# rhasspy/piper

Measured on AMD Instinct MI355X. Metric: audio samples/sec, higher is better.
Workload: dtype f32; 1 GPU; BASELINE configs[1]: medium VITS voice (22050 Hz), 1 utterance(s) x 128 phoneme ids per step per GPU, scales 0.667/1.0/0.8; step = inferSeconds span: host ids in (pe_upload) + pe_run, engine draws both noise sites + int16 PCM to host (pe_fetch); parallelism=utterance-parallel x1, one process per GPU, RCCL weight broadcast

## Files before the change

__graft_entry__.py:

```python
import os
import subprocess
import sys

ROOT = os.path.dirname(os.path.abspath(__file__))
if ROOT not in sys.path:
    sys.path.insert(0, ROOT)


def build() -> None:
    subprocess.check_call(["make", "-C", ROOT, "-j", str(min(8, os.cpu_count() or 1)), "all"])
    try:
        subprocess.check_call(["make", "-C", ROOT, "-j", str(min(8, os.cpu_count() or 1)), "emu"])
    except Exception as e:
        print("emulator build skipped:", e)
    import piper_amd
    from piper_amd import _lib
    lib = _lib.get_lib()
    for s in _lib.SYMBOLS:
        getattr(lib, s)


def smoke() -> None:
    import numpy as np
    from oracle import vits_oracle as O
    from piper_amd import weights as W
    from piper_amd.engine import Engine

    cfg = W.preset("tiny")
    w = W.synthetic_weights(cfg, 1234)
    eng = Engine(blob=W.pack_blob(cfg, w), device=0)
    T = 24
    ids = W.synthetic_phoneme_ids(T, 0, id_max=cfg.n_vocab - 1)
    rng = np.random.default_rng(7)
    nw = rng.standard_normal((2, T)).astype(np.float32)
    nz = rng.standard_normal((cfg.inter, 32 * T + 64)).astype(np.float32)
    scales = (0.667, 1.0, 0.8)
    r = eng.synthesize(ids, scales, noise_w=nw, noise_z=nz)
    o = O.synthesize(w, cfg, ids, scales, nw, nz)
    assert np.array_equal(eng.durations(), o["durations"]), "integer durations differ from the oracle"
    d = (r.pcm[0].astype(np.float64) - o["pcm"].astype(np.float64)) / 32767.0
    rms = float(np.sqrt(np.mean(d * d)))
    assert rms <= 1e-3, f"int16 PCM RMS error {rms} > 1e-3"
    print(f"smoke OK: {r.pcm[0].size} samples, pcm rms err {rms:.2e}")


if __name__ == "__main__":
    build()
    if len(sys.argv) > 1 and sys.argv[1] == "smoke":
        smoke()
```

piper_amd/csrc/kernels/col4.h:

```cpp
#pragma once
#include "dds.h"

namespace pe {

__device__ __forceinline__ int c4_tile(int bx, int nx, int P) { return pe_xcd_tile(bx, nx, P); }

constexpr int FFN_MAXS = 16;
constexpr int C4_H = 192, C4_NT = C4_H / 64;
template <int K>
struct Col4W {
  static constexpr int NQ = K / 16;
  static constexpr int KS = K + 4;
  f32x4 w[C4_NT][K / 16];
};
template <int K>
__device__ __forceinline__ void col_gemm4_fetch(Col4W<K>& W, const float* wp4, int nt, int wv, int lane) {
  constexpr int NQ = Col4W<K>::NQ, tile_floats = (K / 4) * 256;
#pragma unroll
  for (int m = 0; m < C4_NT; ++m) {
    const bool live = PE_UNIFORM(m < nt);
    const pe_rowsrc ws = pe_make_row_u(wp4 + (long)(live ? m : 0) * tile_floats, live ? tile_floats : 0);
#pragma unroll
    for (int q = 0; q < NQ; ++q) W.w[m][q] = pe_row_load4(ws, ((NQ * wv + q) * 64 + lane) * 4);
  }
  PE_SCHED_FENCE();
}
template <int K>
__device__ __forceinline__ void col_gemm4_acc(const Col4W<K>& W, const float* YT, f32x4 (&acc)[C4_NT], int wv, int lane) {
  constexpr int NQ = Col4W<K>::NQ, KS = Col4W<K>::KS;
  const float* yp = YT + (lane & 3) * KS + 4 * NQ * wv;
#pragma unroll
  for (int q = 0; q < NQ; ++q) {
    f32x4 yv;
#pragma unroll
    for (int j = 0; j < 4; ++j) yv[j] = yp[4 * q + j];
#pragma unroll
    for (int j = 0; j < 4; ++j)
#pragma unroll
      for (int m = 0; m < C4_NT; ++m) acc[m] = pe_mfma_4x4x1(W.w[m][q][j], yv[j], acc[m]);
  }
}
__device__ __forceinline__ void col_gemm4_zero(f32x4 (&acc)[C4_NT]) {
#pragma unroll
  for (int m = 0; m < C4_NT; ++m)
#pragma unroll
    for (int r = 0; r < 4; ++r) acc[m][r] = 0.f;
}
__device__ __forceinline__ void col_gemm4_put(const f32x4 (&acc)[C4_NT], float* P, int wv, int lane) {
#pragma unroll
  for (int m = 0; m < C4_NT; ++m)
#pragma unroll
    for (int r = 0; r < 4; ++r) P[((wv * C4_NT + m) * 64 + 4 * (lane >> 2) + r) * 4 + (lane & 3)] = acc[m][r];
}
template <int K>
__device__ __forceinline__ void col_gemm4_run(const Col4W<K>& W, const float* YT, float* P, int wv, int lane) {
  f32x4 acc[C4_NT];
  col_gemm4_zero(acc);
  col_gemm4_acc<K>(W, YT, acc, wv, lane);
  col_gemm4_put(acc, P, wv, lane);
}
template <int K, int K2>
__device__ __forceinline__ void col_gemm4_run2(const Col4W<K>& W, const float* YT, const Col4W<K2>& W2, const float* YT2, float* P,
                                               int wv, int lane) {
  f32x4 acc[C4_NT];
  col_gemm4_zero(acc);
  col_gemm4_acc<K>(W, YT, acc, wv, lane);
  col_gemm4_acc<K2>(W2, YT2, acc, wv, lane);
  col_gemm4_put(acc, P, wv, lane);
}
__device__ __forceinline__ float col_gemm4_get(const float* P, int c, int col) {
  const int o = c * 4 + col;
  return ((P[o] + P[C4_H * 4 + o]) + P[2 * C4_H * 4 + o]) + P[3 * C4_H * 4 + o];
}
__device__ __forceinline__ float pe_col_sum4(float v, float* red, int& flip, int wv, int lane, int col) {
  v += __shfl_xor(v, 4);
  v += __shfl_xor(v, 8);
  v += __shfl_xor(v, 16);
  v += __shfl_xor(v, 32);
  float* r = red + flip * 16;
  flip ^= 1;
  if (lane < 4) r[wv * 4 + col] = v;
  __syncthreads();
  return ((r[col] + r[4 + col]) + r[8 + col]) + r[12 + col];
}


template <bool FRONT>
__global__ __launch_bounds__(256) void colchain4_kernel(const int* lens, const float* in1, long in1_bs, int nx, int xcd, int mode,
                                                        int in1_cs, int K1r, int rows1, int first, int out_cs, ColP p) {
  PE_KTRACE(3);
  constexpr int NC = 4, NVT = 3, K1 = C4_H, K2 = C4_H / 2, KS1 = Col4W<K1>::KS, KS2 = Col4W<K2>::KS;
  PE_DYN_SMEM(float, sm);
  if constexpr (!FRONT) PE_STAMP(3, 0);
  p.lens = lens; p.xcd = xcd; p.mode = mode; p.in1 = in1; p.in1_bs = in1_bs; p.in1_cs = in1_cs; p.K1 = K1r; p.rows1 = rows1;
  p.first = first; p.out_cs = out_cs;
  const int b = blockIdx.y;
  int L = PE_UNIFORM(lens[b]);
  if constexpr (FRONT) PE_ENTRY_BATCH(L, p.res, p.res_bs, p.res_cs, p.gamma, p.beta, p.out, p.out_bs, p.x1, p.x1_bs, p.x1_cs, p.b1, p.w1,
                                      p.in0, p.in0_bs, p.in0_cs, p.w0, p.b0, p.w2, p.b2, p.rows2, p.out2, p.o2_bs, p.o2_cs);
  else PE_ENTRY_BATCH(L, p.res, p.res_bs, p.res_cs, p.gamma, p.beta, p.out, p.out_bs, p.x1, p.x1_bs, p.x1_cs, p.b1, p.w1,
                      p.in0, p.in0_bs, p.in0_cs, p.w2, p.b2, p.kT, p.kt_bs, p.vQ);
  const int t0 = c4_tile(blockIdx.x, nx, p.xcd) * NC;
  if (t0 >= L) return;
  if constexpr (!FRONT) PE_STAMP(3, 1);
  float* YT = sm;
  float* P = YT + NC * KS1;
  float* red = P + 4 * C4_H * NC;
  const int tid = threadIdx.x, col = tid & 3, rl = tid >> 2, wv = PE_UNIFORM(tid >> 6), lane = tid & 63;
  const int t = t0 + col;
  const bool ok = t < L;
  const int part = p.mode >= 2 ? (int)blockIdx.z : 0, row0 = part * C4_H;
  const int rows_here = p.rows1 - row0 < C4_H ? p.rows1 - row0 : C4_H;
  const bool nomain = p.mode == 1 && !p.w1;
  Col4W<K1> gw0;
  Col4W<K1> gw;
  auto fetch_gw = [&]() { col_gemm4_fetch<K1>(gw, p.w1 + (long)part * C4_NT * (K1 / 4) * 256, (rows_here + 63) / 64, wv, lane); };
  const bool skip_part = p.mode == 2 && (p.rows1 <= C4_H || part == 1);
  const bool pre_part = !FRONT && p.mode == 2 && p.w2 && !skip_part;
  float* YTP = P + 4 * C4_H * NC + 32 + 64 * 4;
  Col4W<K2> gw2;
  const bool second = p.mode == 1 && p.w2;
  auto chain_tail = [&](auto m_of, const float* ovv) {
    float* xb = p.x1 + (long)b * p.x1_bs;
    float* YT2 = YT;
    const pe_rowsrc b2d = pe_make_row(second ? p.b2 : p.w1, (second && p.b2) ? p.rows2 : 0);
    float b2v[NVT];
#pragma unroll
    for (int k = 0; k < NVT; ++k) b2v[k] = pe_row_load(b2d, rl + 64 * k);
#pragma unroll
    for (int k = 0; k < NVT; ++k) {
      const int c = rl + 64 * k;
      if (c < K2) {
        const float xn = (ok && c < p.rows1) ? ovv[k] - m_of(k, c) : 0.f;
        if (ok && c < p.rows1) xb[(long)c * p.x1_cs + t] = xn;
        YT2[col * KS2 + c] = xn;
      }
    }
    if (!second) return;
    __syncthreads();
    col_gemm4_run<K2>(gw2, YT2, P, wv, lane);
    __syncthreads();
    if (!ok) return;
    float* o2 = p.out2 + (long)b * p.o2_bs;
#pragma unroll
    for (int k = 0; k < NVT; ++k) {
      const int c = rl + 64 * k;
      if (c < p.rows2) o2[(long)c * p.o2_cs + t] = col_gemm4_get(P, c, col) + b2v[k];
    }
  };
  if (nomain) {
    const pe_rowsrc s0 = pe_make_row(p.in1 + (long)b * p.in1_bs, (FRONT && p.first) ? 0 : K2 * p.in1_cs);
    const pe_rowsrc x1d = pe_make_row(p.x1 + (long)b * p.x1_bs, K2 * p.x1_cs);
    float m[NVT], ovn[NVT];
    m[2] = ovn[2] = 0.f;
    if constexpr (FRONT) {
      const pe_rowsrc a0 = pe_make_row(p.in0 + (long)b * p.in0_bs, K1 * p.in0_cs);
      const pe_rowsrc b0d = pe_make_row(p.b0 ? p.b0 : p.w0, p.b0 ? K2 : 0);
      float av[NVT], b0v[2];
#pragma unroll
      for (int k = 0; k < NVT; ++k) av[k] = pe_row_load(a0, ok ? (rl + 64 * k) * p.in0_cs + t : -1);
#pragma unroll
      for (int k = 0; k < 2; ++k) {
        const int c = rl + 64 * k;
        m[k] = pe_row_load(s0, (ok && c < K2) ? c * p.in1_cs + t : -1);
        b0v[k] = pe_row_load(b0d, c);
        ovn[k] = pe_row_load(x1d, (ok && c < K2) ? c * p.x1_cs + t : -1);
      }
      PE_SCHED_FENCE();
      col_gemm4_fetch<K1>(gw0, p.w0, (K2 + 63) / 64, wv, lane);
#pragma unroll
      for (int k = 0; k < NVT; ++k) YT[col * KS1 + rl + 64 * k] = av[k];
      __syncthreads();
      if (second) col_gemm4_fetch<K2>(gw2, p.w2, (p.rows2 + 63) / 64, wv, lane);
      col_gemm4_run<K1>(gw0, YT, P, wv, lane);
      __syncthreads();
#pragma unroll
      for (int k = 0; k < 2; ++k) m[k] = ok ? (col_gemm4_get(P, rl + 64 * k, col) + b0v[k]) + m[k] : 0.f;
    } else {
#pragma unroll
      for (int k = 0; k < 2; ++k) {
        const int c = rl + 64 * k;
        m[k] = pe_row_load(s0, (ok && c < K2) ? c * p.in1_cs + t : -1);
        ovn[k] = pe_row_load(x1d, (ok && c < K2) ? c * p.x1_cs + t : -1);
      }
      PE_SCHED_FENCE();
      if (second) col_gemm4_fetch<K2>(gw2, p.w2, (p.rows2 + 63) / 64, wv, lane);
    }
    chain_tail([&](int k, int) { return m[k]; }, ovn);
    return;
  }
  float sk[NVT];
  if constexpr (FRONT) {
    const pe_rowsrc a0 = pe_make_row(p.in0 + (long)b * p.in0_bs, K1 * p.in0_cs);
    const pe_rowsrc s0 = pe_make_row(p.in1 + (long)b * p.in1_bs, p.first ? 0 : K1 * p.in1_cs);
    const pe_rowsrc b0d = pe_make_row(p.b0 ? p.b0 : p.w0, p.b0 ? K1 : 0);
    float av[NVT], b0v[NVT];
#pragma unroll
    for (int k = 0; k < NVT; ++k) {
      const int c = rl + 64 * k;
      av[k] = pe_row_load(a0, ok ? c * p.in0_cs + t : -1);
      sk[k] = pe_row_load(s0, ok ? c * p.in1_cs + t : -1);
      b0v[k] = pe_row_load(b0d, c);
    }
    PE_SCHED_FENCE();
    col_gemm4_fetch<K1>(gw0, p.w0, C4_NT, wv, lane);
#pragma unroll
    for (int k = 0; k < NVT; ++k) YT[col * KS1 + rl + 64 * k] = av[k];
    __syncthreads();
    fetch_gw();
    col_gemm4_run<K1>(gw0, YT, P, wv, lane);
    __syncthreads();
#pragma unroll
    for (int k = 0; k < NVT; ++k) sk[k] = ok ? (col_gemm4_get(P, rl + 64 * k, col) + b0v[k]) + sk[k] : 0.f;
  }

  float ov[NVT], gg[NVT], bb[NVT], b1v[NVT];
  {
    const pe_rowsrc ind = pe_make_row(p.in1 + (long)b * p.in1_bs, p.K1 * p.in1_cs);
    const float* obp = p.mode == 0 ? p.res + (long)b * p.res_bs : (skip_part ? p.out + (long)b * p.out_bs : p.x1 + (long)b * p.x1_bs);
    const int ocs = p.mode == 0 ? p.res_cs : (skip_part ? p.out_cs : p.x1_cs);
    const pe_rowsrc od = p.mode == 3 ? pe_make_row(p.res ? p.res + (long)b * p.res_bs + row0 : p.w1, p.res ? rows_here : 0)
                         : pre_part  ? pe_make_row(p.b2 ? p.b2 : p.w1, p.b2 ? rows_here : 0)
                                     : pe_make_row(obp, (skip_part && p.first) ? 0 : rows_here * ocs);
    const pe_rowsrc x0d = pe_make_row(p.in0 + (long)b * p.in0_bs, pre_part ? K2 * p.in0_cs : 0);
    float x0v[2];
    const pe_rowsrc gd = pe_make_row(p.mode == 0 ? p.gamma : p.w1, p.mode == 0 ? p.rows1 : 0);
    const pe_rowsrc bd = pe_make_row(p.mode == 0 ? p.beta : p.w1, p.mode == 0 ? p.rows1 : 0);
    const pe_rowsrc b1d = pe_make_row(p.b1 ? p.b1 + row0 : p.w1, p.b1 ? rows_here : 0);
    float xin[NVT];
#pragma unroll
    for (int k = 0; k < NVT; ++k) {
      const int c = rl + 64 * k;
      xin[k] = FRONT ? sk[k] : pe_row_load(ind, ok ? c * p.in1_cs + t : -1);
      ov[k] = pe_row_load(od, (ok && c < rows_here) ? ((p.mode == 3 || pre_part) ? c : c * ocs + t) : -1);
      if (!FRONT && k < 2) x0v[k] = pe_row_load(x0d, (ok && c < K2) ? c * p.in0_cs + t : -1);
      gg[k] = pe_row_load(gd, c < rows_here ? c : -1);
      bb[k] = pe_row_load(bd, c < rows_here ? c : -1);
      b1v[k] = pe_row_load(b1d, c < rows_here ? c : -1);
    }
    PE_SCHED_FENCE();
    if constexpr (!FRONT) fetch_gw();
    if (pre_part) col_gemm4_fetch<K2>(gw2, p.w2, C4_NT, wv, lane);
    if constexpr (!FRONT) PE_STAMP(3, 2);
#pragma unroll
    for (int k = 0; k < NVT; ++k) YT[col * KS1 + rl + 64 * k] = xin[k];
    if constexpr (!FRONT)
      if (pre_part) {
        YTP[col * KS2 + rl] = x0v[0];
        if (rl < K2 - 64) YTP[col * KS2 + rl + 64] = x0v[1];
      }
  }
  __syncthreads();
  if (pre_part) col_gemm4_run2<K1, K2>(gw, YT, gw2, YTP, P, wv, lane);
  else col_gemm4_run<K1>(gw, YT, P, wv, lane);
  if (second) col_gemm4_fetch<K2>(gw2, p.w2, (p.rows2 + 63) / 64, wv, lane);
  __syncthreads();

  if (p.mode >= 2) {
    if (!ok) return;
    float* tp = (skip_part || p.mode == 3) ? p.out + (long)b * p.out_bs + (p.mode == 3 ? (long)row0 * p.out_cs : 0) : p.x1 + (long)b * p.x1_bs;
    const int tcs = (skip_part || p.mode == 3) ? p.out_cs : p.x1_cs;
#pragma unroll
    for (int k = 0; k < NVT; ++k) {
      const int c = rl + 64 * k;
      if (c < rows_here) {
        const float val = (col_gemm4_get(P, c, col) + b1v[k]) + ov[k];
        tp[(long)c * tcs + t] = val;
        if (p.mode == 3 && p.kT && part == 1) p.kT[(long)b * p.kt_bs + ((long)(c >> 2) * p.out_cs + t) * 4 + (c & 3)] = val;
        if (p.mode == 3 && p.vQ && part == 2) p.vQ[(long)b * p.kt_bs + ((long)(t >> 2) * C4_H + c) * 4 + (t & 3)] = val;
      }
    }
    return;
  }
  if (p.mode == 0) {
    int red_flip = 0;
    auto col_sum = [&](float x) -> float { return pe_col_sum4(x, red, red_flip, wv, lane, col); };
    const int H = p.rows1;
    float v[NVT];
    float s = 0.f;
#pragma unroll
    for (int k = 0; k < NVT; ++k) {
      const int c = rl + 64 * k;
      v[k] = (ok && c < H) ? (col_gemm4_get(P, c, col) + b1v[k]) + ov[k] : 0.f;
      s += v[k];
    }
    const float mean = col_sum(s) / (float)H;
    float q = 0.f;
#pragma unroll
    for (int k = 0; k < NVT; ++k)
      if (rl + 64 * k < H) { const float d = v[k] - mean; q = fmaf(d, d, q); }
    const float rstd = 1.f / sqrtf(col_sum(q) / (float)H + 1e-5f);
    if (!ok) return;
    float* ob = p.out + (long)b * p.out_bs;
#pragma unroll
    for (int k = 0; k < NVT; ++k) {
      const int c = rl + 64 * k;
      if (c < H) ob[(long)c * p.out_cs + t] = (v[k] - mean) * rstd * gg[k] + bb[k];
    }
    return;
  }

  chain_tail([&](int k, int c) { return col_gemm4_get(P, c, col) + b1v[k]; }, ov);
}

__global__ __launch_bounds__(256) void lngemm4_kernel(const int* lens, int nx, int xcd, const float* in, long in_bs, int in_cs,
                                                      int rows, const float* parts, int nparts, LnGemmP p) {
  PE_KTRACE(7);
  constexpr int NC = 4, NVT = 3, H = C4_H, KS = Col4W<H>::KS;
  PE_DYN_SMEM(float, sm);
  p.lens = lens; p.xcd = xcd; p.in = in; p.in_bs = in_bs; p.in_cs = in_cs; p.rows = rows; p.parts = parts; p.nparts = nparts;
  const int b = blockIdx.y;
  int L = PE_UNIFORM(lens[b]);
  PE_ENTRY_BATCH(L, p.gamma, p.beta, p.bias, p.pbias, p.p_bs, p.w16);
  const int t0 = c4_tile(blockIdx.x, nx, p.xcd) * NC;
  if (t0 >= L) return;
  float* YT = sm;
  float* P = YT + NC * KS;
  float* red = P + 4 * H * NC;
  const int tid = threadIdx.x, col = tid & 3, rl = tid >> 2, wv = PE_UNIFORM(tid >> 6), lane = tid & 63;
  const int t = t0 + col;
  const bool ok = t < L;
  const int part = blockIdx.z, row0 = part * H;
  const int rows_here = p.rows - row0 < H ? p.rows - row0 : H;
  Col4W<H> gw;
  auto fetch_gw = [&]() { col_gemm4_fetch<H>(gw, p.w16 + (long)part * C4_NT * (H / 4) * 256, (rows_here + 63) / 64, wv, lane); };
  float v[NVT], gg[NVT], bb[NVT], cb[NVT];
  {
    const pe_rowsrc ind = pe_make_row(p.in + (long)b * p.in_bs, H * p.in_cs);
    const pe_rowsrc gd = pe_make_row(p.gamma, H), bd = pe_make_row(p.beta, H);
    const pe_rowsrc cbd = pe_make_row(p.bias ? p.bias + row0 : p.gamma, p.bias ? rows_here : 0);
#pragma unroll
    for (int k = 0; k < NVT; ++k) {
      const int c = rl + 64 * k;
      v[k] = pe_row_load(ind, ok ? c * p.in_cs + t : -1);
      gg[k] = pe_row_load(gd, c);
      bb[k] = pe_row_load(bd, c);
      cb[k] = pe_row_load(cbd, c);
    }
    if (p.parts) {
      const pe_rowsrc pbd = pe_make_row(p.pbias, H);
      float pv[NVT][FFN_MAXS];
      float pbv[NVT];
#pragma unroll
      for (int k = 0; k < NVT; ++k) {
        const int c = rl + 64 * k;
        pbv[k] = pe_row_load(pbd, c);
        const pe_rowsrc pd = pe_make_row(p.parts + (long)b * p.p_bs + (long)(t0 >> 2) * p.nparts * (H * 4), p.nparts * (H * 4));
#pragma unroll
        for (int sl = 0; sl < FFN_MAXS; ++sl) pv[k][sl] = pe_row_load(pd, (ok && sl < p.nparts) ? sl * (H * 4) + c * 4 + col : -1);
      }
      PE_SCHED_FENCE();
      fetch_gw();
#pragma unroll
      for (int k = 0; k < NVT; ++k) {
        float a = pv[k][0];
#pragma unroll
        for (int sl = 1; sl < FFN_MAXS; ++sl) a += pv[k][sl];
        v[k] = ok ? v[k] + (a + pbv[k]) : 0.f;
      }
    } else {
      PE_SCHED_FENCE();
      fetch_gw();
    }
  }
  int red_flip = 0;
  auto col_sum = [&](float x) -> float { return pe_col_sum4(x, red, red_flip, wv, lane, col); };
  float s = 0.f;
#pragma unroll
  for (int k = 0; k < NVT; ++k) s += v[k];
  const float mean = col_sum(s) / (float)H;
  float q = 0.f;
#pragma unroll
  for (int k = 0; k < NVT; ++k) { const float d = v[k] - mean; q = fmaf(d, d, q); }
  const float rstd = 1.f / sqrtf(col_sum(q) / (float)H + 1e-5f);
  float* xo = p.xout + (long)b * p.x_bs;
#pragma unroll
  for (int k = 0; k < NVT; ++k) {
    const int c = rl + 64 * k;
    const float y = ok ? (v[k] - mean) * rstd * gg[k] + bb[k] : 0.f;
    YT[col * KS + c] = y;
    if (part == 0 && ok) xo[(long)c * p.x_cs + t] = y;
  }
  __syncthreads();
  col_gemm4_run<H>(gw, YT, P, wv, lane);
  __syncthreads();
  if (!ok) return;
  const bool second = p.out2 != nullptr && row0 >= p.split;
  float* ob = second ? p.out2 + (long)b * p.o2_bs + (long)(row0 - p.split) * p.o2_cs : p.out + (long)b * p.o_bs + (long)row0 * p.o_cs;
  const int ocs = second ? p.o2_cs : p.o_cs;
  const pe_rowsrc c2d = pe_make_row((second && p.bias2) ? p.bias2 + (long)b * p.bias2_bs + (row0 - p.split) : p.gamma, (second && p.bias2) ? rows_here : 0);
#pragma unroll
  for (int k = 0; k < NVT; ++k) {
    const int c = rl + 64 * k;
    if (c < rows_here) {
      const float val = (col_gemm4_get(P, c, col) + cb[k]) + pe_row_load(c2d, c);
      ob[(long)c * ocs + t] = val;
      if (p.kT && part == 1) p.kT[(long)b * p.kt_bs + ((long)(c >> 2) * p.x_cs + t) * 4 + (c & 3)] = val;
      if (p.vQ && part == 2) p.vQ[(long)b * p.kt_bs + ((long)(t >> 2) * H + c) * 4 + (t & 3)] = val;
    }
  }
}

}
```

piper_amd/csrc/kernels/launch_front.cpp:

```cpp
#include "launch.h"

#include "attention.h"
#include "attno.h"
#include "attn4.h"
#include "colchain.h"
#include "dds.h"
#include "dds4.h"
#include "ffn.h"
#include "duration.h"
#include "layernorm.h"
#include "glue.h"
#include "spline.h"
#include "timing.h"

namespace pe {
namespace launch {

void init_front() {
#ifndef PE_EMU
  const int lim = 160 * 1024;
  const void* ks[] = {(const void*)attn_kernel<0>, (const void*)attn_kernel<48>, (const void*)attn_kernel<96>,
                      (const void*)attno_kernel<96>, (const void*)attn4_kernel<96, false>, (const void*)attn4_kernel<96, true>};
  for (const void* k : ks) PE_HIP(hipFuncSetAttribute(k, hipFuncAttributeMaxDynamicSharedMemorySize, lim));
#endif
}

void embed(dim3 grid, hipStream_t stream, const EmbedP& p) {
  PE_LAUNCH(embed_kernel, grid, dim3(64), 0, stream, p);
}

void attention(int dk, dim3 grid, size_t smem, hipStream_t stream, const AttnP& p) {
  if (p.sglobal) {
    if (dk == 96) PE_LAUNCH(attn_long_kernel<96>, grid, dim3(256), smem, stream, p);
    else if (dk == 48) PE_LAUNCH(attn_long_kernel<48>, grid, dim3(256), smem, stream, p);
    else PE_LAUNCH(attn_long_kernel<0>, grid, dim3(256), smem, stream, p);
    return;
  }
  if (dk == 96) PE_LAUNCH(attn_kernel<96>, grid, dim3(256), smem, stream, p);
  else if (dk == 48) PE_LAUNCH(attn_kernel<48>, grid, dim3(256), smem, stream, p);
  else PE_LAUNCH(attn_kernel<0>, grid, dim3(256), smem, stream, p);
}

void attno(dim3 grid, size_t smem, hipStream_t stream, const AttnOP& p) {
  PE_LAUNCH(attno_kernel<96>, grid, dim3(512), smem, stream, p);
}

void attn4(bool long_rows, dim3 grid, size_t smem, hipStream_t stream, const AttnOP& p) {
  if (long_rows) PE_LAUNCH((attn4_kernel<96, true>), grid, dim3(256), smem, stream, p.lens, p.qkv, p.q_bs, p.kT, p.kt_bs, (int)grid.x, p.xcd, p.q_cs, p.window, p);
  else PE_LAUNCH((attn4_kernel<96, false>), grid, dim3(256), smem, stream, p.lens, p.qkv, p.q_bs, p.kT, p.kt_bs, (int)grid.x, p.xcd, p.q_cs, p.window, p);
}

void layer_norm(dim3 grid, hipStream_t stream, const LnP& p) { PE_LAUNCH(ln_kernel, grid, dim3(256), 0, stream, p); }

void dds_layer(int nchunks, dim3 grid, size_t smem, hipStream_t stream, const DdsP& p) {
  if (nchunks == 3) PE_LAUNCH(dds_layer16_kernel<3>, grid, dim3(512), smem, stream, p);
  else if (nchunks == 6) PE_LAUNCH(dds_layer16_kernel<6>, grid, dim3(512), smem, stream, p);
  else PE_LAUNCH(dds_layer16_kernel<8>, grid, dim3(512), smem, stream, p);
}

void dds_layer4(dim3 grid, size_t smem, hipStream_t stream, const DdsP& p) {
  PE_LAUNCH(dds_layer4_kernel, grid, dim3(256), smem, stream, p.lens, p.z_scale, (int)grid.x, p.xcd, p.x, p.x_bs, p.x_cs, p.dw_k, p.dw_dil, p);
}

void colchain(dim3 grid, size_t smem, hipStream_t stream, const ColP& p) {
  PE_LAUNCH(colchain_kernel<6>, grid, dim3(512), smem, stream, p);
}

void lngemm(dim3 grid, size_t smem, hipStream_t stream, const LnGemmP& p) {
  PE_LAUNCH(lngemm_kernel<6>, grid, dim3(512), smem, stream, p);
}

void colchain4(dim3 grid, size_t smem, hipStream_t stream, const ColP& p) {
  if (p.w0) PE_LAUNCH(colchain4_kernel<true>, grid, dim3(256), smem, stream, p.lens, p.in1, p.in1_bs, (int)grid.x, p.xcd, p.mode, p.in1_cs, p.K1, p.rows1, p.first, p.out_cs, p);
  else PE_LAUNCH(colchain4_kernel<false>, grid, dim3(256), smem, stream, p.lens, p.in1, p.in1_bs, (int)grid.x, p.xcd, p.mode, p.in1_cs, p.K1, p.rows1, p.first, p.out_cs, p);
}

void lngemm4(dim3 grid, size_t smem, hipStream_t stream, const LnGemmP& p) {
  PE_LAUNCH(lngemm4_kernel, grid, dim3(256), smem, stream, p.lens, (int)grid.x, p.xcd, p.in, p.in_bs, p.in_cs, p.rows, p.parts, p.nparts, p);
}

void ffn(dim3 grid, size_t smem, hipStream_t stream, const FfnP& p) {
  PE_LAUNCH(ffn_kernel, grid, dim3(256), smem, stream, p.lens, p.xcd, (int)grid.x, (int)grid.y, p.x, p.x_bs, p.x_cs, p.w1p, p);
}

void xcc_probe(hipStream_t stream, int* out64) { PE_LAUNCH(xcc_probe_kernel, dim3(64), dim3(64), 0, stream, out64); }

void cf_pre(dim3 grid, hipStream_t stream, const float* z0, long z_bs, const float* w, const float* bias, const float* xg,
            long g_bs, int g_cs, float* out, long o_bs, int o_cs, const int* lens, int H) {
  PE_LAUNCH(cf_pre_kernel, grid, dim3(64), 0, stream, z0, z_bs, w, bias, xg, g_bs, g_cs, out, o_bs, o_cs, lens, H);
}

void spline_inverse(dim3 grid, hipStream_t stream, const float* hproj, long h_bs, int h_cs, float* z1, long z_bs,
                    const int* lens, float inv_sqrt_h) {
  PE_LAUNCH(spline_inverse_kernel, grid, dim3(64), 0, stream, hproj, h_bs, h_cs, z1, z_bs, lens, inv_sqrt_h);
}

void scale(dim3 grid, hipStream_t stream, const float* in, float* out, long n, const float* s, long per_utt) {
  PE_LAUNCH(scale_kernel, grid, dim3(256), 0, stream, in, out, n, s, per_utt);
}

void duration(dim3 grid, hipStream_t stream, const DurP& p) { PE_LAUNCH(duration_kernel, grid, dim3(256), 0, stream, p); }

void duration_plan(dim3 grid, hipStream_t stream, const PlanP& p) { PE_LAUNCH(duration_plan_kernel, grid, dim3(256), 0, stream, p); }

void randn(hipStream_t stream, float* out, long rows, int cols, long stride, long row0, const unsigned long long* state,
           int site, const unsigned long long* keys, const int* use, int ch) {
  PE_LAUNCH(randn_kernel, dim3(randn_blocks(rows, cols)), dim3(256), 0, stream, out, rows, cols, stride, row0, state, site, keys, use,
            ch);
}

void regulate(dim3 grid, hipStream_t stream, const RegP& p) {
  PE_LAUNCH(regulate_kernel, grid, dim3(256), 0, stream, p.absmax, p.tlens, p.rng, p.gen, p.C, p.fold, p);
}

void cond(dim3 grid, hipStream_t stream, const float* emb_g, int gin, const int* sids, const float* w, const float* bias,
          int rows, float* out, int o_bs) {
  PE_LAUNCH(cond_kernel, grid, dim3(128), 0, stream, emb_g, gin, sids, w, bias, rows, out, o_bs);
}

void speaker_blend(hipStream_t stream, int batch, const BlendP& p) {
  PE_LAUNCH(speaker_blend_kernel, dim3((unsigned)((p.gin + 63) / 64), (unsigned)batch), dim3(64), 0, stream, p);
}

}
}

#ifdef PE_STAMPS
PE_TRACE_FETCHER(front)
#endif
```

Before: 126.5 million samples/s.

## Hoist activation and weight loads ahead of entry batch wait in colchain4/lngemm4

```diff
diff --git a/__graft_entry__.py b/__graft_entry__.py
--- a/__graft_entry__.py
+++ b/__graft_entry__.py
@@ -8,9 +8,9 @@
 
 
 def build() -> None:
-    subprocess.check_call(["make", "-C", ROOT, "-j", str(min(8, os.cpu_count() or 1)), "all"])
+    subprocess.check_call(["make", "-C", ROOT, "-j", str(min(8, os.cpu_count() or 1)), "all", "entry1"])
     try:
-        subprocess.check_call(["make", "-C", ROOT, "-j", str(min(8, os.cpu_count() or 1)), "emu"])
+        subprocess.check_call(["make", "-C", ROOT, "-j", str(min(8, os.cpu_count() or 1)), "emu", "emu_entry1"])
     except Exception as e:
         print("emulator build skipped:", e)
     import piper_amd
diff --git a/piper_amd/csrc/kernels/col4.h b/piper_amd/csrc/kernels/col4.h
--- a/piper_amd/csrc/kernels/col4.h
+++ b/piper_amd/csrc/kernels/col4.h
@@ -85,38 +85,89 @@
 }
 
 
+constexpr int C4_F_HPRE = 4;
+constexpr int C4_F_NOMAIN = 8;
+#ifdef PE_ENTRY1_COL4
+constexpr bool C4_ENTRY2 = false;
+#else
+constexpr bool C4_ENTRY2 = true;
+#endif
+constexpr bool C4_EARLY_W = C4_ENTRY2;
 template <bool FRONT>
+#ifdef PE_ENTRY1_COL4
 __global__ __launch_bounds__(256) void colchain4_kernel(const int* lens, const float* in1, long in1_bs, int nx, int xcd, int mode,
                                                         int in1_cs, int K1r, int rows1, int first, int out_cs, ColP p) {
+#else
+__global__ __launch_bounds__(256) void colchain4_kernel(const int* lens, const float* a, long a_bs, const float* wa, int nx, int xcd,
+                                                        int mflags, int a_cs, int K1r, int rows1, ColP p) {
+#endif
   PE_KTRACE(3);
   constexpr int NC = 4, NVT = 3, K1 = C4_H, K2 = C4_H / 2, KS1 = Col4W<K1>::KS, KS2 = Col4W<K2>::KS;
   PE_DYN_SMEM(float, sm);
   if constexpr (!FRONT) PE_STAMP(3, 0);
+#ifdef PE_ENTRY1_COL4
   p.lens = lens; p.xcd = xcd; p.mode = mode; p.in1 = in1; p.in1_bs = in1_bs; p.in1_cs = in1_cs; p.K1 = K1r; p.rows1 = rows1;
   p.first = first; p.out_cs = out_cs;
+  const bool nomain_f = false, hpre_f = false;
+#else
+  p.lens = lens; p.xcd = xcd; p.mode = mflags & 3; p.K1 = K1r; p.rows1 = rows1;
+  if constexpr (FRONT) { p.in0 = a; p.in0_bs = a_bs; p.in0_cs = a_cs; p.w0 = wa; }
+  else { p.in1 = a; p.in1_bs = a_bs; p.in1_cs = a_cs; p.w1 = wa; }
+  const bool nomain_f = (mflags & C4_F_NOMAIN) != 0, hpre_f = (mflags & C4_F_HPRE) != 0;
+#endif
   const int b = blockIdx.y;
   int L = PE_UNIFORM(lens[b]);
-  if constexpr (FRONT) PE_ENTRY_BATCH(L, p.res, p.res_bs, p.res_cs, p.gamma, p.beta, p.out, p.out_bs, p.x1, p.x1_bs, p.x1_cs, p.b1, p.w1,
-                                      p.in0, p.in0_bs, p.in0_cs, p.w0, p.b0, p.w2, p.b2, p.rows2, p.out2, p.o2_bs, p.o2_cs);
-  else PE_ENTRY_BATCH(L, p.res, p.res_bs, p.res_cs, p.gamma, p.beta, p.out, p.out_bs, p.x1, p.x1_bs, p.x1_cs, p.b1, p.w1,
-                      p.in0, p.in0_bs, p.in0_cs, p.w2, p.b2, p.kT, p.kt_bs, p.vQ);
+  if constexpr (!C4_ENTRY2) {
+    if constexpr (FRONT) PE_ENTRY_BATCH(L, p.res, p.res_bs, p.res_cs, p.gamma, p.beta, p.out, p.out_bs, p.x1, p.x1_bs, p.x1_cs, p.b1, p.w1,
+                                        p.in0, p.in0_bs, p.in0_cs, p.w0, p.b0, p.w2, p.b2, p.rows2, p.out2, p.o2_bs, p.o2_cs);
+    else PE_ENTRY_BATCH(L, p.res, p.res_bs, p.res_cs, p.gamma, p.beta, p.out, p.out_bs, p.x1, p.x1_bs, p.x1_cs, p.b1, p.w1,
+                        p.in0, p.in0_bs, p.in0_cs, p.w2, p.b2, p.kT, p.kt_bs, p.vQ);
+  }
   const int t0 = c4_tile(blockIdx.x, nx, p.xcd) * NC;
-  if (t0 >= L) return;
-  if constexpr (!FRONT) PE_STAMP(3, 1);
+  if constexpr (!C4_ENTRY2) {
+    if (t0 >= L) return;
+    if constexpr (!FRONT) PE_STAMP(3, 1);
+  }
   float* YT = sm;
   float* P = YT + NC * KS1;
   float* red = P + 4 * C4_H * NC;
   const int tid = threadIdx.x, col = tid & 3, rl = tid >> 2, wv = PE_UNIFORM(tid >> 6), lane = tid & 63;
   const int t = t0 + col;
-  const bool ok = t < L;
+  bool ok = false;
+  if constexpr (!C4_ENTRY2) ok = t < L;
   const int part = p.mode >= 2 ? (int)blockIdx.z : 0, row0 = part * C4_H;
   const int rows_here = p.rows1 - row0 < C4_H ? p.rows1 - row0 : C4_H;
-  const bool nomain = p.mode == 1 && !p.w1;
+  const bool nomain = p.mode == 1 && (C4_ENTRY2 ? nomain_f : !p.w1);
   Col4W<K1> gw0;
   Col4W<K1> gw;
   auto fetch_gw = [&]() { col_gemm4_fetch<K1>(gw, p.w1 + (long)part * C4_NT * (K1 / 4) * 256, (rows_here + 63) / 64, wv, lane); };
+  float xe[NVT];
+  bool gw_early = false;
+  if constexpr (C4_ENTRY2) {
+    const float* ea = FRONT ? p.in0 : p.in1;
+    const long ea_bs = FRONT ? p.in0_bs : p.in1_bs;
+    const int ea_cs = FRONT ? p.in0_cs : p.in1_cs;
+    const pe_rowsrc ed = pe_make_row(ea + (long)b * ea_bs, (FRONT ? K1 : p.K1) * ea_cs);
+#pragma unroll
+    for (int k = 0; k < NVT; ++k) xe[k] = pe_row_load(ed, (rl + 64 * k) * ea_cs + t);
+    PE_SCHED_FENCE();
+    if constexpr (FRONT) {
+      col_gemm4_fetch<K1>(gw0, p.w0, nomain ? (K2 + 63) / 64 : C4_NT, wv, lane);
+    } else if (!nomain && !hpre_f) {
+      fetch_gw();
+      gw_early = true;
+    }
+    if constexpr (FRONT) PE_ENTRY_BATCH(L, p.res, p.res_bs, p.res_cs, p.gamma, p.beta, p.out, p.out_bs, p.x1, p.x1_bs, p.x1_cs, p.b1, p.w1,
+                                        p.in1, p.in1_bs, p.in1_cs, p.first, p.b0, p.w2, p.b2, p.rows2, p.out2, p.o2_bs, p.o2_cs);
+    else PE_ENTRY_BATCH(L, p.res, p.res_bs, p.res_cs, p.gamma, p.beta, p.out, p.out_bs, p.out_cs, p.first, p.x1, p.x1_bs, p.x1_cs, p.b1,
+                        p.in0, p.in0_bs, p.in0_cs, p.w2, p.b2, p.kT, p.kt_bs, p.vQ);
+    if (t0 >= L) return;
+    ok = t < L;
+#pragma unroll
+    for (int k = 0; k < NVT; ++k) xe[k] = ok ? xe[k] : 0.f;
+  }
   const bool skip_part = p.mode == 2 && (p.rows1 <= C4_H || part == 1);
-  const bool pre_part = !FRONT && p.mode == 2 && p.w2 && !skip_part;
+  const bool pre_part =!FRONT && p.mode == 2 && p.w2 && !skip_part;
   float* YTP = P + 4 * C4_H * NC + 32 + 64 * 4;
   Col4W<K2> gw2;
   const bool second = p.mode == 1 && p.w2;
@@ -158,7 +209,7 @@
       const pe_rowsrc b0d = pe_make_row(p.b0 ? p.b0 : p.w0, p.b0 ? K2 : 0);
       float av[NVT], b0v[2];
 #pragma unroll
-      for (int k = 0; k < NVT; ++k) av[k] = pe_row_load(a0, ok ? (rl + 64 * k) * p.in0_cs + t : -1);
+      for (int k = 0; k < NVT; ++k) av[k] = C4_ENTRY2 ? xe[k] : pe_row_load(a0, ok ? (rl + 64 * k) * p.in0_cs + t : -1);
 #pragma unroll
       for (int k = 0; k < 2; ++k) {
         const int c = rl + 64 * k;
@@ -167,7 +218,7 @@
         ovn[k] = pe_row_load(x1d, (ok && c < K2) ? c * p.x1_cs + t : -1);
       }
       PE_SCHED_FENCE();
-      col_gemm4_fetch<K1>(gw0, p.w0, (K2 + 63) / 64, wv, lane);
+      if constexpr (!C4_EARLY_W) col_gemm4_fetch<K1>(gw0, p.w0, (K2 + 63) / 64, wv, lane);
 #pragma unroll
       for (int k = 0; k < NVT; ++k) YT[col * KS1 + rl + 64 * k] = av[k];
       __syncthreads();
@@ -180,7 +231,7 @@
 #pragma unroll
       for (int k = 0; k < 2; ++k) {
         const int c = rl + 64 * k;
-        m[k] = pe_row_load(s0, (ok && c < K2) ? c * p.in1_cs + t : -1);
+        m[k] = C4_ENTRY2 ? xe[k] : pe_row_load(s0, (ok && c < K2) ? c * p.in1_cs + t : -1);
         ovn[k] = pe_row_load(x1d, (ok && c < K2) ? c * p.x1_cs + t : -1);
       }
       PE_SCHED_FENCE();
@@ -198,12 +249,12 @@
 #pragma unroll
     for (int k = 0; k < NVT; ++k) {
       const int c = rl + 64 * k;
-      av[k] = pe_row_load(a0, ok ? c * p.in0_cs + t : -1);
+      av[k] = C4_ENTRY2 ? xe[k] : pe_row_load(a0, ok ? c * p.in0_cs + t : -1);
       sk[k] = pe_row_load(s0, ok ? c * p.in1_cs + t : -1);
       b0v[k] = pe_row_load(b0d, c);
     }
     PE_SCHED_FENCE();
-    col_gemm4_fetch<K1>(gw0, p.w0, C4_NT, wv, lane);
+    if constexpr (!C4_EARLY_W) col_gemm4_fetch<K1>(gw0, p.w0, C4_NT, wv, lane);
 #pragma unroll
     for (int k = 0; k < NVT; ++k) YT[col * KS1 + rl + 64 * k] = av[k];
     __syncthreads();
@@ -231,7 +282,7 @@
 #pragma unroll
     for (int k = 0; k < NVT; ++k) {
       const int c = rl + 64 * k;
-      xin[k] = FRONT ? sk[k] : pe_row_load(ind, ok ? c * p.in1_cs + t : -1);
+      xin[k] = FRONT ? sk[k] : (C4_ENTRY2 ? xe[k] : pe_row_load(ind, ok ? c * p.in1_cs + t : -1));
       ov[k] = pe_row_load(od, (ok && c < rows_here) ? ((p.mode == 3 || pre_part) ? c : c * ocs + t) : -1);
       if (!FRONT && k < 2) x0v[k] = pe_row_load(x0d, (ok && c < K2) ? c * p.in0_cs + t : -1);
       gg[k] = pe_row_load(gd, c < rows_here ? c : -1);
@@ -239,7 +290,8 @@
       b1v[k] = pe_row_load(b1d, c < rows_here ? c : -1);
     }
     PE_SCHED_FENCE();
-    if constexpr (!FRONT) fetch_gw();
+    if constexpr (!FRONT)
+      if (!gw_early) fetch_gw();
     if (pre_part) col_gemm4_fetch<K2>(gw2, p.w2, C4_NT, wv, lane);
     if constexpr (!FRONT) PE_STAMP(3, 2);
 #pragma unroll
@@ -303,29 +355,88 @@
   chain_tail([&](int k, int c) { return col_gemm4_get(P, c, col) + b1v[k]; }, ov);
 }
 
+#ifdef PE_ENTRY1_LNGEMM4
+constexpr bool LG4_ENTRY2 = false;
 __global__ __launch_bounds__(256) void lngemm4_kernel(const int* lens, int nx, int xcd, const float* in, long in_bs, int in_cs,
                                                       int rows, const float* parts, int nparts, LnGemmP p) {
+#else
+constexpr bool LG4_ENTRY2 = true;
+__global__ __launch_bounds__(256) void lngemm4_kernel(const int* lens, const float* in, const float* parts, const float* pbias,
+                                                      int in_bs, int in_cs, int p_bs, int nxp, int rows, LnGemmP p) {
+#endif
   PE_KTRACE(7);
   constexpr int NC = 4, NVT = 3, H = C4_H, KS = Col4W<H>::KS;
   PE_DYN_SMEM(float, sm);
+#ifdef PE_ENTRY1_LNGEMM4
   p.lens = lens; p.xcd = xcd; p.in = in; p.in_bs = in_bs; p.in_cs = in_cs; p.rows = rows; p.parts = parts; p.nparts = nparts;
+#else
+  const int nx = nxp & 0xffff;
+  p.lens = lens; p.xcd = (nxp >> 16) & 0xff; p.in = in; p.in_bs = in_bs; p.in_cs = in_cs; p.rows = rows; p.parts = parts;
+  p.nparts = (nxp >> 24) & 0x7f; p.pbias = pbias; p.p_bs = p_bs;
+#endif
   const int b = blockIdx.y;
   int L = PE_UNIFORM(lens[b]);
-  PE_ENTRY_BATCH(L, p.gamma, p.beta, p.bias, p.pbias, p.p_bs, p.w16);
+  if constexpr (!LG4_ENTRY2) PE_ENTRY_BATCH(L, p.gamma, p.beta, p.bias, p.pbias, p.p_bs, p.w16);
   const int t0 = c4_tile(blockIdx.x, nx, p.xcd) * NC;
-  if (t0 >= L) return;
+  if constexpr (!LG4_ENTRY2)
+    if (t0 >= L) return;
   float* YT = sm;
   float* P = YT + NC * KS;
   float* red = P + 4 * H * NC;
   const int tid = threadIdx.x, col = tid & 3, rl = tid >> 2, wv = PE_UNIFORM(tid >> 6), lane = tid & 63;
   const int t = t0 + col;
-  const bool ok = t < L;
+  bool ok = false;
+  if constexpr (!LG4_ENTRY2) ok = t < L;
   const int part = blockIdx.z, row0 = part * H;
   const int rows_here = p.rows - row0 < H ? p.rows - row0 : H;
   Col4W<H> gw;
   auto fetch_gw = [&]() { col_gemm4_fetch<H>(gw, p.w16 + (long)part * C4_NT * (H / 4) * 256, (rows_here + 63) / 64, wv, lane); };
   float v[NVT], gg[NVT], bb[NVT], cb[NVT];
-  {
+  if constexpr (LG4_ENTRY2) {
+    const pe_rowsrc ind = pe_make_row(p.in + (long)b * p.in_bs, H * p.in_cs);
+    float pv[NVT][FFN_MAXS];
+    float pbv[NVT];
+#pragma unroll
+    for (int k = 0; k < NVT; ++k) v[k] = pe_row_load(ind, (rl + 64 * k) * p.in_cs + t);
+    if (p.parts) {
+      const pe_rowsrc pbd = pe_make_row(p.pbias, H);
+      const pe_rowsrc pd = pe_make_row(p.parts + (long)b * p.p_bs + (long)(t0 >> 2) * p.nparts * (H * 4), p.nparts * (H * 4));
+#pragma unroll
+      for (int k = 0; k < NVT; ++k) {
+        const int c = rl + 64 * k;
+        pbv[k] = pe_row_load(pbd, c);
+#pragma unroll
+        for (int sl = 0; sl < FFN_MAXS; ++sl) pv[k][sl] = pe_row_load(pd, sl < p.nparts ? sl * (H * 4) + c * 4 + col : -1);
+      }
+    }
+    PE_SCHED_FENCE();
+    PE_ENTRY_BATCH(L, p.gamma, p.beta, p.bias, p.w16);
+    if (t0 >= L) return;
+    ok = t < L;
+    const pe_rowsrc gd = pe_make_row(p.gamma, H), bd = pe_make_row(p.beta, H);
+    const pe_rowsrc cbd = pe_make_row(p.bias ? p.bias + row0 : p.gamma, p.bias ? rows_here : 0);
+#pragma unroll
+    for (int k = 0; k < NVT; ++k) {
+      const int c = rl + 64 * k;
+      gg[k] = pe_row_load(gd, c);
+      bb[k] = pe_row_load(bd, c);
+      cb[k] = pe_row_load(cbd, c);
+    }
+    PE_SCHED_FENCE();
+    fetch_gw();
+    if (p.parts) {
+#pragma unroll
+      for (int k = 0; k < NVT; ++k) {
+        float a = pv[k][0];
+#pragma unroll
+        for (int sl = 1; sl < FFN_MAXS; ++sl) a += pv[k][sl];
+        v[k] = ok ? v[k] + (a + pbv[k]) : 0.f;
+      }
+    } else {
+#pragma unroll
+      for (int k = 0; k < NVT; ++k) v[k] = ok ? v[k] : 0.f;
+    }
+  } else {
     const pe_rowsrc ind = pe_make_row(p.in + (long)b * p.in_bs, H * p.in_cs);
     const pe_rowsrc gd = pe_make_row(p.gamma, H), bd = pe_make_row(p.beta, H);
     const pe_rowsrc cbd = pe_make_row(p.bias ? p.bias + row0 : p.gamma, p.bias ? rows_here : 0);
diff --git a/piper_amd/csrc/kernels/launch_front.cpp b/piper_amd/csrc/kernels/launch_front.cpp
--- a/piper_amd/csrc/kernels/launch_front.cpp
+++ b/piper_amd/csrc/kernels/launch_front.cpp
@@ -71,12 +71,29 @@
 }
 
 void colchain4(dim3 grid, size_t smem, hipStream_t stream, const ColP& p) {
+#ifndef PE_ENTRY1_COL4
+  const int mflags = p.mode | ((p.mode == 2 && p.w2) ? C4_F_HPRE : 0) | ((p.mode == 1 && !p.w1) ? C4_F_NOMAIN : 0);
+  if (p.mode < 0 || p.mode > 3) throw std::runtime_error("internal: colchain4 mode");
+  if (p.w0) PE_LAUNCH(colchain4_kernel<true>, grid, dim3(256), smem, stream, p.lens, p.in0, p.in0_bs, p.w0, (int)grid.x, p.xcd, mflags, p.in0_cs, p.K1, p.rows1, p);
+  else PE_LAUNCH(colchain4_kernel<false>, grid, dim3(256), smem, stream, p.lens, p.in1, p.in1_bs, p.w1, (int)grid.x, p.xcd, mflags, p.in1_cs, p.K1, p.rows1, p);
+  return;
+#else
   if (p.w0) PE_LAUNCH(colchain4_kernel<true>, grid, dim3(256), smem, stream, p.lens, p.in1, p.in1_bs, (int)grid.x, p.xcd, p.mode, p.in1_cs, p.K1, p.rows1, p.first, p.out_cs, p);
   else PE_LAUNCH(colchain4_kernel<false>, grid, dim3(256), smem, stream, p.lens, p.in1, p.in1_bs, (int)grid.x, p.xcd, p.mode, p.in1_cs, p.K1, p.rows1, p.first, p.out_cs, p);
+#endif
 }
 
 void lngemm4(dim3 grid, size_t smem, hipStream_t stream, const LnGemmP& p) {
+#ifndef PE_ENTRY1_LNGEMM4
+  auto fits31 = [](long v) { return v >= 0 && v <= 0x7fffffffL; };
+  if (!fits31(p.in_bs) || !fits31(p.p_bs)) throw std::runtime_error("internal: lngemm4 batch stride does not fit 32 bits");
+  if (grid.x > 0xffffu || p.xcd < 0 || p.xcd > 0xff || p.nparts < 0 || p.nparts > 0x7f)
+    throw std::runtime_error("internal: lngemm4 grid width / XCD count / slice count does not fit its packed parameter");
+  const int nxp = (int)grid.x | (p.xcd << 16) | (p.nparts << 24);
+  PE_LAUNCH(lngemm4_kernel, grid, dim3(256), smem, stream, p.lens, p.in, p.parts, p.pbias, (int)p.in_bs, p.in_cs, (int)p.p_bs, nxp, p.rows, p);
+#else
   PE_LAUNCH(lngemm4_kernel, grid, dim3(256), smem, stream, p.lens, (int)grid.x, p.xcd, p.in, p.in_bs, p.in_cs, p.rows, p.parts, p.nparts, p);
+#endif
 }
 
 void ffn(dim3 grid, size_t smem, hipStream_t stream, const FfnP& p) {
```

New measurement: 126.9 million samples/s, median of 6. No clear change (+0.3%).
